# sinamalakouti/CDDMSL

Hardware: AMD Instinct MI355X
Metric: images/sec (train step) VOC+Clipart RN50-C4 (higher is better)
Workload: dtype bf16

## Files before the change

### cddmsl_amd/csrc/elementwise.hip

```cpp
#include "common.h"
#include <stdlib.h>

namespace {

template <typename T> struct Elt;
template <> struct Elt<__bf16> {
  static constexpr int ES = 2, VEC = 8;
  __device__ static __forceinline__ void unpack(const u32x4& v, float* f) {
#pragma unroll
    for (int j = 0; j < 4; ++j) { f[2 * j] = bf2f(v[j] & 0xffff); f[2 * j + 1] = bf2f(v[j] >> 16); }
  }
  __device__ static __forceinline__ u32x4 pack(const float* f) {
    u32x4 v;
#pragma unroll
    for (int j = 0; j < 4; ++j) v[j] = pack2bf(f[2 * j], f[2 * j + 1]);
    return v;
  }
  __device__ static __forceinline__ float ld(const char* p) { return bf2f(*(const unsigned short*)p); }
  __device__ static __forceinline__ void st(char* p, float v) { *(unsigned short*)p = f2bf(v); }
};
template <> struct Elt<float> {
  static constexpr int ES = 4, VEC = 4;
  __device__ static __forceinline__ void unpack(const u32x4& v, float* f) {
    const f32x4 x = __builtin_bit_cast(f32x4, v);
    f[0] = x[0]; f[1] = x[1]; f[2] = x[2]; f[3] = x[3];
  }
  __device__ static __forceinline__ u32x4 pack(const float* f) {
    f32x4 x = {f[0], f[1], f[2], f[3]};
    return __builtin_bit_cast(u32x4, x);
  }
  __device__ static __forceinline__ float ld(const char* p) { return *(const float*)p; }
  __device__ static __forceinline__ void st(char* p, float v) { *(float*)p = v; }
};

template <typename T>
__device__ __forceinline__ void preprocess_px(const unsigned char* img, char* out, int n, int h, int w, int Hp, int Wp, int Cp,
                                              float m0, float m1, float m2, float s0, float s1, float s2, float div) {
  long i = (long)blockIdx.x * blockDim.x + threadIdx.x;
  if (i >= (long)Hp * Wp) return;
  const unsigned ii = (unsigned)i;
  int x = ii % (unsigned)Wp, y = ii / (unsigned)Wp;
  float v[3] = {0.f, 0.f, 0.f};
  if (y < h && x < w) {
    long o = (long)y * w + x, pl = (long)h * w;
    v[0] = ((float)img[o] / div - m0) / s0;
    v[1] = ((float)img[pl + o] / div - m1) / s1;
    v[2] = ((float)img[2 * pl + o] / div - m2) / s2;
  }
  char* dst = out + (((long)n * Hp + y) * Wp + x) * Cp * Elt<T>::ES;
  if (Cp == Elt<T>::VEC) {
    float o[8] = {v[0], v[1], v[2], 0.f, 0.f, 0.f, 0.f, 0.f};
    *(u32x4*)dst = Elt<T>::pack(o);
    return;
// ... 320 lines not shown
  }
}

template <typename T>
__global__ void k_attnpool_softmax_fwd(const float* S, float* p, char* pT, long rows, int H, int P1, int TP, float scale) {
  const long r = (long)blockIdx.x * blockDim.x + threadIdx.x;
  if (r >= rows) return;
  const long k = r / H; const int h = (int)(r - k * H);
  const float* s = S + r * TP;
  float mx = -INFINITY;
  for (int t = 0; t < P1; ++t) mx = fmaxf(mx, s[t] * scale);
  float sum = 0.f;
  for (int t = 0; t < P1; ++t) sum += expf(s[t] * scale - mx);
  const float inv = 1.f / sum;
  for (int t = 0; t < TP; ++t) {
    float v = 0.f;
    if (t < P1) { v = expf(s[t] * scale - mx) * inv; p[r * P1 + t] = v; }
    Elt<T>::st(pT + ((k * TP + t) * H + h) * Elt<T>::ES, v);
  }
}
template <typename T>
__global__ void k_attnpool_softmax_bwd(const float* p, const float* dP, char* dsT, char* pds, long rows, int H, int P1, int TP,
                                       float scale) {
  const long r = (long)blockIdx.x * blockDim.x + threadIdx.x;
  if (r >= rows) return;
  const long k = r / H; const int h = (int)(r - k * H);
  const float* pr = p + r * P1;
  const float* dp = dP + r * TP;
  float dot = 0.f;
  for (int t = 0; t < P1; ++t) dot += pr[t] * dp[t];
  char* prow = pds + ((k * 2 * H + h) * TP) * Elt<T>::ES;
  char* drow = pds + ((k * 2 * H + H + h) * TP) * Elt<T>::ES;
  for (int t = 0; t < TP; ++t) {
    float pv = 0.f, ds = 0.f;
    if (t < P1) { pv = pr[t]; ds = pv * (dp[t] - dot) * scale; }
    Elt<T>::st(dsT + ((k * TP + t) * H + h) * Elt<T>::ES, ds);
    Elt<T>::st(prow + t * Elt<T>::ES, pv);
    Elt<T>::st(drow + t * Elt<T>::ES, ds);
  }
}

template <typename T>
__global__ __launch_bounds__(256) void k_attnpool_softmax_fwd_w(const float* __restrict__ S, float* __restrict__ p, char* __restrict__ pT,
                                                                long K, int H, int P1, int TP, float scale) {
  const long k = (long)blockIdx.x * 4 + (threadIdx.x >> 6);
  const int t = threadIdx.x & 63;
  if (k >= K) return;
  float v[32];
#pragma unroll
  for (int h = 0; h < 32; ++h) {
    v[h] = 0.f;
    if (h < H) {
      const bool in = t < P1;
      const float x = in ? S[(k * H + h) * TP + t] * scale : -INFINITY;
      const float mx = wave_max(x);
      const float e = in ? expf(x - mx) : 0.f;
      const float sum = wave_sum(e);
      v[h] = e * (1.f / sum);
      if (in) p[(k * H + h) * P1 + t] = v[h];
    }
  }
  if (t < TP) {
    char* dst = pT + ((k * TP + t) * H) * Elt<T>::ES;
    if (H % Elt<T>::VEC == 0) {
#pragma unroll
      for (int g = 0; g < 32 / Elt<T>::VEC; ++g)
        if (g * Elt<T>::VEC < H) ((u32x4*)dst)[g] = Elt<T>::pack(v + g * Elt<T>::VEC);
    } else {
#pragma unroll
      for (int h = 0; h < 32; ++h)
        if (h < H) Elt<T>::st(dst + h * Elt<T>::ES, v[h]);
    }
  }
}
template <typename T>
__global__ __launch_bounds__(256) void k_attnpool_softmax_bwd_w(const float* __restrict__ p, const float* __restrict__ dP,
                                                                char* __restrict__ dsT, char* __restrict__ pds, long K, int H, int P1,
                                                                int TP, float scale) {
  const long k = (long)blockIdx.x * 4 + (threadIdx.x >> 6);
  const int t = threadIdx.x & 63;
  if (k >= K) return;
  float dsv[32];
#pragma unroll
  for (int h = 0; h < 32; ++h) {
    dsv[h] = 0.f;
    if (h < H) {
      const bool in = t < P1;
      const float pv = in ? p[(k * H + h) * P1 + t] : 0.f;
      const float dp = in ? dP[(k * H + h) * TP + t] : 0.f;
      const float dot = wave_sum(pv * dp);
      dsv[h] = in ? pv * (dp - dot) * scale : 0.f;
      if (t < TP) {
        Elt<T>::st(pds + ((k * 2 * H + h) * TP + t) * Elt<T>::ES, pv);
        Elt<T>::st(pds + ((k * 2 * H + H + h) * TP + t) * Elt<T>::ES, dsv[h]);
      }
    }
  }
  if (t < TP) {
    char* dst = dsT + ((k * TP + t) * H) * Elt<T>::ES;
    if (H % Elt<T>::VEC == 0) {
#pragma unroll
      for (int g = 0; g < 32 / Elt<T>::VEC; ++g)
        if (g * Elt<T>::VEC < H) ((u32x4*)dst)[g] = Elt<T>::pack(dsv + g * Elt<T>::VEC);
    } else {
#pragma unroll
      for (int h = 0; h < 32; ++h)
        if (h < H) Elt<T>::st(dst + h * Elt<T>::ES, dsv[h]);
    }
  }
}

template <typename T>
__global__ void k_relu_bwd(const char* g, const char* y, char* dx, long nchunks, int g_f32) {
  for (long i = (long)blockIdx.x * blockDim.x + threadIdx.x; i < nchunks; i += (long)gridDim.x * blockDim.x) {
    float a[8], m[8], o[8];
    Elt<T>::unpack(((const u32x4*)y)[i], m);
    if (g_f32 && Elt<T>::VEC == 8) {
      Elt<float>::unpack(((const u32x4*)g)[2 * i], a);
      Elt<float>::unpack(((const u32x4*)g)[2 * i + 1], a + 4);
    } else Elt<T>::unpack(((const u32x4*)g)[i], a);
#pragma unroll
    for (int j = 0; j < Elt<T>::VEC; ++j) o[j] = m[j] > 0.f ? a[j] : 0.f;
    ((u32x4*)dx)[i] = Elt<T>::pack(o);
  }
}

template <typename T>
__global__ void k_colsum(const char* x, float* out, long rows, int cols, int period, int slab) {
  int c = blockIdx.x * 64 + (threadIdx.x & 63);
  int rlane = threadIdx.x >> 6;
  int res = blockIdx.z;
  long j0 = (long)blockIdx.y * slab;
  long nj = (rows - res + period - 1) / period;
  float s = 0.f;
  if (c < cols)
    for (long j = j0 + rlane; j < min(nj, j0 + slab); j += 4) s += Elt<T>::ld(x + ((res + period * j) * cols + c) * Elt<T>::ES);
  __shared__ float red[4][64];
  red[rlane][threadIdx.x & 63] = s;
  __syncthreads();
  if (rlane == 0 && c < cols) atomicAdd(out + (long)res * cols + c, red[0][threadIdx.x] + red[1][threadIdx.x] + red[2][threadIdx.x] + red[3][threadIdx.x]);
}

template <typename T>
__global__ void k_colsum_vec(const char* x, float* out, long rows, int cols, int period, int slab) {
// ... 469 lines not shown
```

### cddmsl_amd/hip.py

```python
import ctypes
import math
import os
from ctypes import c_float, c_int, c_long, c_void_p

import torch

from ._lib import check, lib, ptr, require_cuda, stream_ptr

DT = {torch.bfloat16: 0, torch.float32: 1}

_sigs_done = False


def _L():
    global _sigs_done
    L = lib()
    if not _sigs_done:
        vp, ci, cf = c_void_p, c_int, c_float
        L.cddmsl_last_kernel.argtypes = []
        L.cddmsl_plan_only.argtypes = [ci]
        L.cddmsl_conv_fwd.argtypes = [vp] * 7 + [ci] * 16 + [vp]
        L.cddmsl_bottleneck64_ok.argtypes = [ci] * 4
        L.cddmsl_bottleneck64_fwd.argtypes = [vp] * 17 + [ci] * 4 + [vp]
        L.cddmsl_conv_wgrad.argtypes = [vp] * 4 + [ci] * 12 + [vp]
        L.cddmsl_set_workspace.argtypes = [vp, c_long]
        L.cddmsl_weight_prep.argtypes = [vp] * 4 + [ci] * 5 + [vp]
        L.cddmsl_weight_prep_multi.argtypes = [vp, ci, ci, vp]
        L.cddmsl_preprocess.argtypes = [vp, vp] + [ci] * 6 + [vp, vp, ci, ci, vp]
        L.cddmsl_maxpool3s2_fwd.argtypes = [vp, vp] + [ci] * 5 + [vp]
        L.cddmsl_upsample_zero2.argtypes = [vp] * 4 + [ci] * 5 + [vp]
        L.cddmsl_meanpool_fwd.argtypes = [vp, vp, c_long, ci, ci, ci, vp]
        L.cddmsl_meanpool_bwd.argtypes = [vp, vp, c_long, ci, ci, ci, vp]
        L.cddmsl_preprocess224.argtypes = [vp, vp] + [ci] * 11 + [vp, vp, ci, vp]
        L.cddmsl_preprocess_batch.argtypes = [vp, vp, vp, ci, vp, ci, ci, ci, vp, vp, ci, ci, vp]
        L.cddmsl_preprocess224_batch.argtypes = [vp, vp, vp, ci, vp] + [ci] * 8 + [vp, vp, ci, vp]
        L.cddmsl_tta_view.argtypes = [vp] + [ci] * 4 + [vp, vp, vp, ci] * 2 + [vp, ci, ci, ci] * 2 + [ci, vp, vp, ci, ci, vp]
        L.cddmsl_resize_batch_u8.argtypes = [vp, c_long, vp, c_long, vp, c_long, vp, ci, vp]
        L.cddmsl_avgpool2_fwd.argtypes = [vp, vp] + [ci] * 5 + [vp]
        L.cddmsl_avgpool2_bwd.argtypes = [vp] * 4 + [ci] * 5 + [vp]
        L.cddmsl_avgpool2_bwd_q8.argtypes = [vp] * 4 + [ci] * 4 + [vp] * 4
        L.cddmsl_avgpool2_fwd_bits.argtypes = [vp] * 3 + [ci] * 5 + [vp]
        L.cddmsl_avgpool2_bwd_bits.argtypes = [vp] * 3 + [ci] * 5 + [vp]
        L.cddmsl_conv3x3_pool_fwd.argtypes = [vp] * 6 + [ci] * 7 + [vp]
        L.cddmsl_attn_tokens_fwd.argtypes = [vp] * 3 + [ci] * 5 + [vp]
        L.cddmsl_attn_tokens_bwd.argtypes = [vp] * 4 + [ci] * 5 + [vp]
        L.cddmsl_attnpool_softmax_fwd.argtypes = [vp] * 3 + [c_long, ci, ci, ci, cf, ci, vp]
        L.cddmsl_attnpool_softmax_bwd.argtypes = [vp] * 4 + [c_long, ci, ci, ci, cf, ci, vp]
        L.cddmsl_gemm_nt_batched.argtypes = [vp] * 4 + [ci] * 7 + [c_long] * 3 + [ci, ci, vp]
        L.cddmsl_gemm_tn_batched.argtypes = [vp] * 3 + [ci] * 7 + [c_long] * 3 + [ci, ci, vp]
        L.cddmsl_relu_bwd.argtypes = [vp, vp, vp, c_long, ci, ci, vp]
        L.cddmsl_colsum.argtypes = [vp, vp, c_long, ci, ci, ci, vp]
        L.cddmsl_sgd_clip_step.argtypes = [vp] * 4 + [ci, vp] + [cf] * 4 + [ci, vp]
        L.cddmsl_sgd_step_groups.argtypes = [vp] * 6 + [ci, vp, cf, ci, ci, cf, ci, vp]
        L.cddmsl_roi_align_forward.argtypes = [vp] * 5 + [ci] * 7 + [cf, ci, ci, ci, vp]
        L.cddmsl_roi_align_backward.argtypes = [vp] * 7 + [ci] * 7 + [cf, ci, ci, ci, vp]
        L.cddmsl_nms_anyorder.argtypes = [vp] * 4 + [ci, cf, vp, vp, vp]
        L.cddmsl_soft_nms.argtypes = [vp] * 6 + [ci, ci, cf, cf, cf, ci, vp, vp, vp]
        L.cddmsl_openset_logits.argtypes = [vp] * 4 + [ci] * 4 + [cf, cf, vp]
        L.cddmsl_openset_select.argtypes = [vp, vp, ci, vp, ci, vp, ci, ci, cf, cf, cf] + [vp] * 6 + [ci, vp, vp, vp]
        L.cddmsl_roi_align_nchw_anyorder.argtypes = [vp] * 3 + [ci] * 7 + [cf, ci, ci, ci, vp, vp, vp]
        L.cddmsl_roi_align_backward_nchw_anyorder.argtypes = [vp] * 3 + [ci] * 7 + [cf, ci, ci, ci, vp, vp, vp]
        L.cddmsl_quantize_fp8.argtypes = [vp] * 4 + [c_long, ci, vp]
        L.cddmsl_conv_fwd_fp8.argtypes = [vp] * 7 + [ci] * 10 + [vp] * 4
        L.cddmsl_conv_wgrad_fp8_ok.argtypes = [ci] * 6
        L.cddmsl_conv_wgrad_fp8.argtypes = [vp] * 4 + [ci] * 9 + [vp]
        L.cddmsl_conv_fwd_q8.argtypes = [vp] * 7 + [ci] * 10 + [vp] * 4
        L.cddmsl_fp8_dot_nt.argtypes = [vp] * 4 + [ci] * 4 + [vp]
        L.cddmsl_roi_align_forward_affine.argtypes = [vp] * 6 + [ci] * 8 + [cf, ci, ci, ci] + [vp] * 4
        L.cddmsl_roi_align_backward_pooled.argtypes = [vp] * 7 + [ci] * 7 + [cf, ci, ci, ci, vp]
        L.cddmsl_anchors.argtypes = [vp, vp, ci, ci, ci, cf, cf, vp]
        L.cddmsl_sort_desc.argtypes = [vp] * 5 + [ci, ci, vp, vp, vp]
        L.cddmsl_rpn_decode.argtypes = [vp] * 6 + [ci] * 5 + [cf] * 8 + [vp]
        L.cddmsl_nms.argtypes = [vp] * 5 + [ci, ci, cf, ci, vp]
        L.cddmsl_iou_match.argtypes = [vp, ci, vp, ci, vp, vp, vp, ci, cf, cf, ci, ci, ci, ci, vp]
        L.cddmsl_iou_match_batched.argtypes = [vp] * 7 + [ci] * 5 + [cf, cf] + [ci] * 4 + [vp]
        L.cddmsl_l2norm_fwd.argtypes = [vp, vp, vp, c_long, ci, cf, vp]
        L.cddmsl_l2norm_bwd.argtypes = [vp, vp, vp, vp, c_long, ci, vp]
        L.cddmsl_cosine_logits_fwd.argtypes = [vp] * 4 + [c_long, ci, ci, cf, cf, vp]
        L.cddmsl_cosine_logits_bwd.argtypes = [vp] * 5 + [c_long, ci, ci, cf, ci, vp]
        L.cddmsl_layernorm_fwd.argtypes = [vp] * 6 + [c_long, ci, cf, ci, vp]
        L.cddmsl_layernorm_bwd.argtypes = [vp] * 6 + [c_long, ci, ci, ci, vp]
        L.cddmsl_layernorm_bwd_emit.argtypes = [vp] * 7 + [c_long, ci, ci, ci, ctypes.POINTER(ci), vp]
        L.cddmsl_focal_ce_fwd.argtypes = [vp] * 4 + [c_long, ci, cf, ci, cf, vp]
        L.cddmsl_focal_ce_bwd.argtypes = [vp] * 5 + [c_long, ci, cf, ci, cf, vp]
        L.cddmsl_attn_small_fwd.argtypes = [vp] * 4 + [ci] * 8 + [cf, ci, vp]
        L.cddmsl_attn_small_bwd.argtypes = [vp] * 7 + [ci] * 8 + [cf, ci, vp]
        L.cddmsl_attn_tokens_fwd_mask.argtypes = [vp] * 4 + [ci] * 5 + [vp]
        L.cddmsl_attnpool_dx.argtypes = [vp] * 6 + [ci] * 6 + [vp]
        L.cddmsl_rpn_losses.argtypes = [vp, vp, vp, ci, vp, ci, vp, vp, vp, vp, c_long, cf, cf, cf, cf, cf, vp, vp, vp, vp, vp]
        L.cddmsl_box_l1.argtypes = [vp, ci, vp, ci, vp, vp, vp, cf, cf, cf, cf, cf, vp, vp, vp, vp]
        L.cddmsl_rpn_losses_reg.argtypes = [vp, vp, vp, ci, vp, ci, vp, vp, vp, vp, c_long, cf, cf, cf, cf, cf, ci, cf, cf, vp, vp, vp, vp, vp]
        L.cddmsl_box_reg_loss.argtypes = [vp, ci, vp, ci, vp, vp, vp, cf, cf, cf, cf, cf, ci, cf, cf, vp, vp, vp, vp]
        L.cddmsl_attn_last_fwd.argtypes = [vp] * 4 + [ci] * 8 + [cf, ci, vp]
        L.cddmsl_attn_last_bwd.argtypes = [vp] * 6 + [ci] * 8 + [cf, ci, vp]
        L.cddmsl_contrastive_fwd.argtypes = [vp] * 4 + [ci, ci, vp]
        L.cddmsl_contrastive_bwd.argtypes = [vp] * 5 + [ci, ci, vp]
        L.cddmsl_instance_boxes.argtypes = [vp] + [ci] * 4 + [vp, ci, vp, vp, vp, vp]
        L.cddmsl_text_embed.argtypes = [vp] * 4 + [c_long, ci, ci, ci, ci, vp]
        L.cddmsl_attn_causal_fwd.argtypes = [vp, vp] + [ci] * 6 + [cf, ci, vp]
        L.cddmsl_quick_gelu.argtypes = [vp, c_long, ci, vp]
# ... 648 lines not shown
def attnpool_dx_ok(K, H, P, TP, C, dtype):
    return dtype == torch.bfloat16 and P == 49 and TP == 56 and 2 * H <= 64 and (2 * H) % 8 == 0 and C % 128 == 0 and 0 < K <= 65535 * 8


@_timed("attnpool_dx")
def attnpool_dx(pds, zu, g0, mbits, P, gpos=None):
    require_cuda(pds, zu, g0, mbits)
    K, H2, TP = pds.shape
    C = zu.shape[2]
    assert pds.dtype == zu.dtype == torch.bfloat16 and g0.dtype == torch.float32 and mbits.dtype == torch.int64
    assert pds.is_contiguous() and zu.is_contiguous() and g0.is_contiguous() and mbits.is_contiguous() and tuple(zu.shape) == (K, H2, C)
    assert tuple(g0.shape) == (K, C) and tuple(mbits.shape) == (K, C) and (gpos is None or (gpos.dtype == torch.float32 and tuple(gpos.shape) == (P + 1, C) and gpos.is_contiguous()))
    dx = torch.empty((K, P, C), device=pds.device, dtype=pds.dtype)
    check(_L().cddmsl_attnpool_dx(ptr(pds), ptr(zu), ptr(g0), ptr(mbits), ptr(dx), ptr(gpos), K, H2, P, TP, C, 0, stream_ptr()), "cddmsl_attnpool_dx")
    return dx


@_timed("attn_tokens_bwd")
def attn_tokens_bwd(dtok, P, relu_mask=None, gpos=None, want_dx=True):
    require_cuda(dtok, relu_mask, gpos)
    K, TP, C = dtok.shape
    assert dtok.is_contiguous()
    assert relu_mask is None or (relu_mask.is_contiguous() and relu_mask.dtype == dtok.dtype and relu_mask.numel() == K * P * C)
    assert gpos is None or (gpos.is_contiguous() and gpos.dtype == torch.float32 and tuple(gpos.shape) == (P + 1, C))
    assert want_dx or gpos is not None
    dx = torch.empty((K, P, C), device=dtok.device, dtype=dtok.dtype) if want_dx else None
    check(_L().cddmsl_attn_tokens_bwd(ptr(dtok), ptr(relu_mask), ptr(dx), ptr(gpos), K, P, TP, C, _dt(dtok), stream_ptr()), "cddmsl_attn_tokens_bwd")
    return dx


@_timed("attnpool_softmax")
def attnpool_softmax_fwd(S, P1, scale, dtype):
    require_cuda(S)
    K, H, TP = S.shape
    assert S.dtype == torch.float32 and S.is_contiguous() and P1 <= TP
    p = torch.empty((K, H, P1), device=S.device, dtype=torch.float32)
    pT = torch.empty((K, TP, H), device=S.device, dtype=dtype)
    check(_L().cddmsl_attnpool_softmax_fwd(ptr(S), ptr(p), ptr(pT), K, H, P1, TP, float(scale), DT[dtype], stream_ptr()), "cddmsl_attnpool_softmax_fwd")
    return p, pT


@_timed("attnpool_softmax")
def attnpool_softmax_bwd(p, dP, scale, dtype):
    require_cuda(p, dP)
    K, H, P1 = p.shape
    TP = dP.shape[2]
    assert p.dtype == dP.dtype == torch.float32 and p.is_contiguous() and dP.is_contiguous() and dP.shape[:2] == (K, H)
    dsT = torch.empty((K, TP, H), device=p.device, dtype=dtype)
    pds = torch.empty((K, 2 * H, TP), device=p.device, dtype=dtype)
    check(_L().cddmsl_attnpool_softmax_bwd(ptr(p), ptr(dP), ptr(dsT), ptr(pds), K, H, P1, TP, float(scale), DT[dtype], stream_ptr()), "cddmsl_attnpool_softmax_bwd")
    return dsT, pds


def _eptr(t, elem_offset=0):
    return ctypes.c_void_p(t.data_ptr() + elem_offset * t.element_size())


@_timed("gemm_nt_batched")
def gemm_nt_batched(a, w, c, M, N, K, lda, ldb, ldc, batch, sa, sw, sc, a_off=0, w_off=0, c_off=0, bias=None):
    require_cuda(a, w, c, bias)
    assert a.dtype == w.dtype and c.dtype in (a.dtype, torch.float32)
    out_f32 = int(c.dtype == torch.float32 and a.dtype != torch.float32)
    check(_L().cddmsl_gemm_nt_batched(_eptr(a, a_off), _eptr(w, w_off), _eptr(c, c_off), ptr(bias), M, N, K, lda, ldb, ldc, batch,
                                      sa, sw, sc, out_f32, _dt(a), stream_ptr()), "cddmsl_gemm_nt_batched")


@_timed("gemm_tn_batched")
def gemm_tn_batched(a, b, out, M, N, K, lda, ldb, ldo, batch, sa, sb, so, a_off=0, b_off=0, o_off=0, accumulate=False):
    require_cuda(a, b, out)
    assert a.dtype == b.dtype
    if accumulate:
        assert out.dtype == torch.float32
        mode = 0
    else:
        mode = 1 if (out.dtype == torch.float32 and a.dtype != torch.float32) else (1 if out.dtype == torch.float32 else 2)
        assert out.dtype in (a.dtype, torch.float32)
    check(_L().cddmsl_gemm_tn_batched(_eptr(a, a_off), _eptr(b, b_off), _eptr(out, o_off), M, N, K, lda, ldb, ldo, batch, sa, sb, so,
                                      mode, _dt(a), stream_ptr()), "cddmsl_gemm_tn_batched")


@_timed("relu_bwd")
def relu_bwd(g, y):
    require_cuda(g, y)
    assert g.is_contiguous() and y.is_contiguous() and g.numel() == y.numel()
    g_f32 = int(g.dtype == torch.float32 and y.dtype != torch.float32)
    assert g_f32 or g.dtype == y.dtype
    dx = torch.empty_like(y)
    check(_L().cddmsl_relu_bwd(ptr(g), ptr(y), ptr(dx), y.numel(), g_f32, _dt(y), stream_ptr()), "cddmsl_relu_bwd")
    return dx


@_timed("colsum")
def colsum(x2d, period=1, out=None):
    require_cuda(x2d, out)
    rows, cols = x2d.shape
    assert x2d.is_contiguous()
    if out is None:
        out = torch.zeros((period, cols) if period > 1 else (cols,), device=x2d.device, dtype=torch.float32)
    check(_L().cddmsl_colsum(ptr(x2d), ptr(out), rows, cols, period, _dt(x2d), stream_ptr()), "cddmsl_colsum")
    return out


def same_layout(a, b):
    return a.shape == b.shape and all(sa == sb for sa, sb, n in zip(a.stride(), b.stride(), a.shape) if n > 1)


# ... 815 lines not shown
```

### cddmsl_amd/layers.py

```python
import os
import weakref

import torch

from . import hip

_STEP = [0]


def bump_weight_version():
    _STEP[0] += 1


_LOAD_GEN = [0]


def note_weights_loaded(*_):
    _LOAD_GEN[0] += 1
    _STEP[0] += 1


def load_generation():
    return _LOAD_GEN[0]

# ... 810 lines not shown
        shape, scale, sr, aligned, K = ctx.meta
        dy = dy.contiguous()
        dx = hip.roi_align_backward(dy[:K], rois, roi_start, shape, scale, sr, aligned)
        dextra = dy[K:] if (dy.shape[0] > K and ctx.needs_input_grad[8]) else None
        return dx, None, None, None, None, None, None, None, dextra


def roi_align(x, rois, roi_start, out_size, scale, sampling_ratio, aligned=True, with_pooled=False, extra=None):
    assert rois.dim() == 2 and rois.size(1) == 5
    assert extra is None or tuple(extra.shape[1:]) == (out_size, out_size, x.shape[3])
    if with_pooled and out_size % 2 == 0:
        y, yp = RoIAlignFn.apply(x, rois, roi_start, out_size, scale, sampling_ratio, aligned, True, extra)
        y._pooled2 = yp
        return y
    return RoIAlignFn.apply(x, rois, roi_start, out_size, scale, sampling_ratio, aligned, False, extra)


class AttnPoolParams:
    def __init__(self, pos, q_w, q_b, k_w, k_b, v_w, v_b, c_w, c_b, heads, frozen=False):
        self.pos, self.heads, self.frozen = pos, heads, frozen
        self.q_w, self.q_b, self.k_w, self.k_b, self.v_w, self.v_b, self.c_w, self.c_b = q_w, q_b, k_w, k_b, v_w, v_b, c_w, c_b
        self.pq = PreparedWeight(q_w, None, frozen)
        self.pk = PreparedWeight(k_w, None, frozen)
        self.pv = PreparedWeight(v_w, None, frozen)
        self.pc = PreparedWeight(c_w, None, frozen)


class AttnPoolFn(torch.autograd.Function):

    TP = 56

    @staticmethod
    def forward(ctx, x, anchor, ap, premask_input_grad=False):
        ctx.relu_src = x if premask_input_grad else None
        T = x.dtype
        K, h, w, C = x.shape
        P, TP, H = h * w, AttnPoolFn.TP, ap.heads
        D = C // H
        assert ap.pos.shape[0] == P + 1 <= TP, "attention pool needs a 7x7 map (clip_backbone.py:86)"
        dev = x.device
        fused_dx = hip.attnpool_dx_ok(K, H, P, TP, C, T) and bool(ctx.needs_input_grad[0]) and os.environ.get("CDDMSL_ATTNPOOL_DX", "1") != "0"
        mbits = None
        if fused_dx and premask_input_grad:
            tok, mbits = hip.attn_tokens_fwd_mask(x.view(K, P, C), ap.pos.detach(), TP)
        else:
            tok = hip.attn_tokens_fwd(x.view(K, P, C), ap.pos.detach(), TP)
        wq, _ = ap.pq.get(T, False)
        wk, wkT = ap.pk.get(T, True)
        wv, wvT = ap.pv.get(T, True)
        wc, _ = ap.pc.get(T, False)
        q0 = hip.conv_fwd(tok.view(K, 1, TP, C), wq, None, ap.q_b.detach(), stride=TP).view(K, C)
        zu = torch.empty((K, 2 * H, C), device=dev, dtype=T)
        hip.gemm_nt_batched(q0, wkT, zu, K, C, D, C, C, 2 * H * C, H, D, D, C, c_off=H * C)
        S = torch.empty((K, H, TP), device=dev, dtype=torch.float32)
        hip.gemm_nt_batched(zu, tok, S, H, TP, C, C, C, TP, K, 2 * H * C, TP * C, H * TP, a_off=H * C)
        p, pT = hip.attnpool_softmax_fwd(S, P + 1, D ** -0.5, T)
        z = torch.empty((K, H, C), device=dev, dtype=T)
        hip.gemm_tn_batched(pT, tok, z, TP, H, C, H, C, C, K, TP * H, TP * C, H * C)
        o = torch.empty((K, C), device=dev, dtype=T)
        hip.gemm_nt_batched(z, wv, o, K, D, C, H * C, C, C, H, C, D * C, D)
        o = o + ap.v_b.detach().to(T)
        out = hip.conv_fwd(o.view(1, 1, K, C), wc, None, ap.c_b.detach(), out_f32=True).view(K, -1)
        ctx.ap = ap
        ctx.fused_dx = fused_dx
        ctx.save_for_backward(tok, q0, zu, p, z, o, mbits)
        ctx.shape = (K, h, w, C)
        return out

    @staticmethod
    def backward(ctx, dout):
        ap = ctx.ap
        tok, q0, zu, p, z, o, mbits = ctx.saved_tensors
        K, h, w, C = ctx.shape
        P, TP, H = h * w, AttnPoolFn.TP, ap.heads
        D = C // H
        T = tok.dtype
        dev = tok.device
        train = not ap.frozen
        dout_t = dout.contiguous().to(T)
        if train:
            hip.conv_wgrad(o.view(1, 1, K, C), dout_t.view(1, 1, K, -1), _ohwi(ap.c_w).shape, out=_ohwi(_grad_buf(ap.c_w)))
            hip.colsum(dout_t, out=_grad_buf(ap.c_b))
        _, wcd = ap.pc.get(T, True)
        wk, wkT = ap.pk.get(T, True)
        wv, wvT = ap.pv.get(T, True)
        do = hip.conv_fwd(dout_t.view(1, 1, K, -1), wcd).view(K, C)
        if train:
            hip.colsum(do, out=_grad_buf(ap.v_b))
            hip.gemm_tn_batched(do, z, _grad_buf(ap.v_w), K, D, C, C, H * C, C, H, D, C, D * C, accumulate=True)
        hip.gemm_nt_batched(do, wvT, zu, K, C, D, C, C, 2 * H * C, H, D, D, C)
        dP = torch.empty((K, H, TP), device=dev, dtype=torch.float32)
        hip.gemm_nt_batched(zu, tok, dP, H, TP, C, C, C, TP, K, 2 * H * C, TP * C, H * TP)
        dsT, pds = hip.attnpool_softmax_bwd(p, dP, D ** -0.5, T)
        du = torch.empty((K, H, C), device=dev, dtype=T)
        hip.gemm_tn_batched(dsT, tok, du, TP, H, C, H, C, C, K, TP * H, TP * C, H * C)
        dq0 = torch.empty((K, C), device=dev, dtype=T)
        hip.gemm_nt_batched(du, wk, dq0, K, D, C, H * C, C, C, H, C, D * C, D)
        if train:
            hip.gemm_tn_batched(q0, du, _grad_buf(ap.k_w), K, D, C, C, H * C, C, H, D, C, D * C, accumulate=True)
            _grad_buf(ap.k_b)
            hip.conv_wgrad(tok.view(K, 1, TP, C), dq0.view(K, 1, 1, C), _ohwi(ap.q_w).shape, stride=TP, out=_ohwi(_grad_buf(ap.q_w)))
            hip.colsum(dq0, out=_grad_buf(ap.q_b))
        _, wqd = ap.pq.get(T, True)
        gpos = _grad_buf(ap.pos) if train else None
        want_dx = ctx.needs_input_grad[0]
        if ctx.fused_dx and want_dx:
            g0 = hip.conv_fwd(dq0.view(1, 1, K, C), wqd, out_f32=True).view(K, C)
            if mbits is None:
                mbits = torch.full((K, C), -1, device=dev, dtype=torch.int64)
            dx = hip.attnpool_dx(pds, zu, g0, mbits, P, gpos)
            return dx.view(K, h, w, C), None, None, None
        dtok = torch.empty((K, TP, C), device=dev, dtype=T)
        hip.gemm_tn_batched(pds, zu, dtok, 2 * H, TP, C, TP, C, C, K, 2 * H * TP, 2 * H * C, TP * C)
        dtok[:, 0, :] += hip.conv_fwd(dq0.view(1, 1, K, C), wqd).view(K, C)
        dx = None
        if want_dx or train:
            dx = hip.attn_tokens_bwd(dtok, P, ctx.relu_src if want_dx else None, gpos, want_dx)
        return (dx.view(K, h, w, C) if want_dx else None), None, None, None


def attnpool(x, ap):
    return AttnPoolFn.apply(x, None if ap.frozen else ap.q_w, ap)


_FP8_CONST = {}


def _fp8_const(value, device):
    k = (float(value), str(device))
    if k not in _FP8_CONST:
        _FP8_CONST[k] = torch.tensor([float(value)], device=device, dtype=torch.float32)
    return _FP8_CONST[k]


def fp8_unit_rows(wn):
    return hip.quantize_fp8(wn.contiguous(), _fp8_const(hip.FP8_MAX, wn.device))


class CosineLogitsFn(torch.autograd.Function):
    @staticmethod
    def forward(ctx, x, wn, temperature, fp8=False, wn8=None):
        x = x.contiguous()
        if fp8 and x.shape[1] % 64 == 0 and wn.shape[0] <= 32:
            xn, inv = hip.l2norm_fwd(x, 1e-12)
            unit = _fp8_const(hip.FP8_MAX, x.device)
            if wn8 is None:
                wn8 = fp8_unit_rows(wn)
            dot = hip.fp8_dot_nt(hip.quantize_fp8(xn, unit), wn8, _fp8_const(1.0 / (hip.FP8_MAX * hip.FP8_MAX * temperature), x.device))
# ... 305 lines not shown
```

### include/cddmsl_hip.h

```cpp
#ifndef CDDMSL_HIP_H
#define CDDMSL_HIP_H
#include <stddef.h>

#ifdef __cplusplus
extern "C" {
#endif

int cddmsl_abi_version(void);

int cddmsl_conv_fwd(const void* x, const void* w, void* y, const float* scale, const float* bias, const void* residual,
                    const void* relu_mask, int Nimg, int Hi, int Wi, int Cin, int Cout, int KH, int KW, int stride, int pad,
                    int pool, int ldy, int ldr, int ldm, int relu, int out_f32, int dtype, void* stream);
int cddmsl_conv3x3_pool_fwd(const void* x, const void* w, void* y, const float* scale, const float* bias, const void* relu_mask,
                            int Nimg, int Hi, int Wi, int Cin, int Cout, int stride, int dtype, void* stream);
int cddmsl_bottleneck64_ok(int Nimg, int H, int W, int dtype);
int cddmsl_bottleneck64_fwd(const void* o1, const void* w2, const float* s2, const float* b2, const void* w3, const float* s3,
                            const float* b3, const void* residual, const void* x0, const void* wd, const float* sd,
                            const float* bd, const void* w1n, const float* s1n, const float* b1n, void* out, void* o1n,
                            int Nimg, int H, int W, int dtype, void* stream);
int cddmsl_set_workspace(void* ptr, long bytes);
int cddmsl_conv_wgrad(const void* x, const void* dy, float* dw, const float* scale, int Nimg, int Hi, int Wi, int Cin,
                      int Cout, int KH, int KW, int stride, int pad, int pool, int ldd, int dtype, void* stream);
int cddmsl_gemm_nt_batched(const void* a, const void* w, void* c, const float* bias, int M, int N, int K, int lda, int ldb, int ldc,
                           int batch, long sa, long sw, long sc, int out_f32, int dtype, void* stream);
// ... 23 lines not shown
                              int* ws_fp, int N, int C, int H, int W, int K, int ph, int pw, float spatial_scale,
                              int sampling_ratio, int aligned, int dtype, void* stream);
int cddmsl_roi_align_forward_affine(const void* x, const float* rois, void* y, void* y_pooled, const float* scale,
                                    const float* bias, int relu, int N, int C, int H, int W, int K, int ph, int pw,
                                    float spatial_scale, int sampling_ratio, int aligned, int dtype, void* y8, const float* q8,
                                    float* amax8, void* stream);
int cddmsl_roi_align_backward_pooled(const void* dy, const float* rois, const int* roi_start, void* dx, float* ws_ay,
                                     float* ws_ax, int* ws_fp, int N, int C, int H, int W, int K, int ph, int pw,
                                     float spatial_scale, int sampling_ratio, int aligned, int dtype, void* stream);
int cddmsl_roi_align_nchw_anyorder(const void* input, const float* rois, void* output, int N, int C, int H, int W, int K, int ph, int pw,
                                   float spatial_scale, int sampling_ratio, int aligned, int dtype, void* temp, size_t* temp_bytes,
                                   void* stream);
int cddmsl_roi_align_backward_nchw_anyorder(const void* grad, const float* rois, void* grad_input, int N, int C, int H, int W, int K,
                                            int ph, int pw, float spatial_scale, int sampling_ratio, int aligned, int dtype, void* temp,
                                            size_t* temp_bytes, void* stream);

int cddmsl_anchors(const float* cell, float* out, int Hf, int Wf, int A, float stride, float offset, void* stream);
int cddmsl_sort_desc(const float* keys_in, float* keys_out, int* idx_scratch, int* order_out, const int* offsets, int N,
                     int total, void* temp, size_t* temp_bytes, void* stream);
int cddmsl_rpn_decode(const int* order, const float* deltas, const float* cell, const int* img_hw, float* boxes,
                      unsigned char* valid, int N, int Hf, int Wf, int A, int topk, float stride, float offset, float wx,
                      float wy, float ww, float wh, float scale_clamp, float min_size, void* stream);
int cddmsl_nms(const float* boxes, const unsigned char* valid, unsigned long long* mask_ws, int* keep, int* nkeep, int N,
               int n, float thr, int max_keep, void* stream);
int cddmsl_nms_anyorder(const float* boxes, const float* scores, long* keep, int* nkeep, int K, float iou_threshold, void* temp,
                        size_t* temp_bytes, void* stream);
int cddmsl_soft_nms(const float* boxes, const float* scores, const long* idxs, long* keep, float* keep_scores, int* nkeep, int K,
                    int method, float sigma, float iou_threshold, float prune_threshold, int max_keep, void* temp,
                    size_t* temp_bytes, void* stream);
int cddmsl_openset_logits(const float* x, const float* wn, float* logits, float* stats, int R, int D, int K, int ld,
                          float temperature, float eps, void* stream);
int cddmsl_openset_select(const float* logits, const float* stats, int ld, const float* boxes, int ldb, const float* objectness,
                          int R, int K, float img_h, float img_w, float score_thresh, int* cand_row, int* cand_cls,
                          float* cand_score, float* cand_box, unsigned char* valid, int* count, int cap, void* temp,
                          size_t* temp_bytes, void* stream);
int cddmsl_iou_match(const float* gt, int G, const float* preds, int P, long* matches, signed char* labels,
                     unsigned int* best_ws, int nthr, float t0, float t1, int l0, int l1, int l2, int allow_low_quality,
                     void* stream);

int cddmsl_iou_match_batched(const float* gt, const int* gt_off, const float* preds, const int* pred_off, long* matches,
                             signed char* labels, unsigned int* best_ws, int N, int P, int maxG, int totalG, int nthr, float t0,
                             float t1, int l0, int l1, int l2, int allow_low_quality, void* stream);

int cddmsl_attn_tokens_fwd(const void* x, const float* pos, void* tok, int K, int P, int TP, int C, int dtype, void* stream);
int cddmsl_attn_tokens_fwd_mask(const void* x, const float* pos, void* tok, unsigned long long* mbits, int K, int P, int TP, int C,
                                int dtype, void* stream);
int cddmsl_attnpool_dx(const void* pds, const void* zu, const float* g0, const unsigned long long* mbits, void* dx, float* gpos, int K,
                       int H2, int P, int TP, int C, int dtype, void* stream);
int cddmsl_attn_tokens_bwd(const void* dtok, const void* relu_mask, void* dx, float* gpos, int K, int P, int TP, int C, int dtype,
                           void* stream);
int cddmsl_attnpool_softmax_fwd(const float* S, float* p, void* pT, long K, int H, int P1, int TP, float scale, int dtype, void* stream);
int cddmsl_attnpool_softmax_bwd(const float* p, const float* dP, void* dsT, void* pds, long K, int H, int P1, int TP, float scale,
                                int dtype, void* stream);

int cddmsl_attn_small_fwd(const void* q, const void* k, const void* v, void* o, int nseq, int t, int heads, int dh, int ldq,
                          int ldk, int ldv, int ldo, float scale, int dtype, void* stream);
int cddmsl_attn_small_bwd(const void* q, const void* k, const void* v, const void* dout, void* dq, void* dk, void* dv, int nseq,
                          int t, int heads, int dh, int ldq, int ldk, int ldv, int ldo, float scale, int dtype, void* stream);
int cddmsl_attn_last_fwd(const void* q, const void* kv, void* o, float* p, int n, int t, int heads, int dh, int ldq, int ldkv, int voff,
                         int ldo, float scale, int dtype, void* stream);
int cddmsl_attn_last_bwd(const void* q, const void* kv, const void* dout, const float* p, void* dq, void* dkv, int n, int t, int heads,
                         int dh, int ldq, int ldkv, int voff, int ldo, float scale, int dtype, void* stream);

int cddmsl_text_embed(const long* ids, const void* tok, const float* pos, float* x, long rows, int t, int W, int vocab, int dtype,
                      void* stream);
int cddmsl_attn_causal_fwd(const void* qkv, void* o, int nseq, int t, int heads, int dh, int ldqkv, int ldo, float scale, int dtype,
                           void* stream);
int cddmsl_quick_gelu(void* x, long numel, int dtype, void* stream);
int cddmsl_text_pool(const float* x, const long* rows, const float* gamma, const float* beta, void* y, long R, int nout, int group,
                     int W, float eps, int dtype, void* stream);

int cddmsl_skinny_gemm_workspace(int M, int N, int K);
int cddmsl_skinny_gemm(const void* x, const void* w, const float* bias, const float* residual, void* y, float* ws, long ws_bytes, int M,
                       int N, int K, int epi, void* stream);
int cddmsl_lm_head_workspace(int M, int V);
int cddmsl_lm_head_argmax(const void* h, const void* wte, long* ids, int ld_ids, float* logits, void* ws, long ws_bytes, int M, int V,
                          int K, void* stream);
int cddmsl_decode_attn(const void* qkv, void* kc, void* vc, void* o, int nseq, int heads, int dh, int L, int Lmax, int ldqkv, float scale,
                       int dtype, void* stream);
int cddmsl_pos_embed(const long* ids, int ld_ids, const void* tab, const float* src, const float* wpe, float* x, long rows, int t, int pos0,
                     int W, int vocab, int npos, int dtype, void* stream);
int cddmsl_gelu_new(void* x, long numel, int dtype, void* stream);
int cddmsl_lm_head_topk_workspace(int M, int V);
int cddmsl_lm_head_topk(const void* h, const void* wte, float* vals, int* idx, float* logZ, float* logits, void* ws, long ws_bytes, int M,
                        int V, int K, int B, void* stream);
int cddmsl_beam_step(const float* vals, const int* idx, const float* logZ, const float* sum_in, const int* len_in,
                     const unsigned char* stop_in, const int* hist_in, const unsigned char* anc_in, float* sum_out, int* len_out,
                     unsigned char* stop_out, int* hist_out, unsigned char* anc_out, int* src, long* next_tok, int n, int B, int T, int step,
                     int stop_id, void* stream);
int cddmsl_decode_attn_beam(const void* qkv, const void* pk, const void* pv, void* gk, void* gv, const unsigned char* anc, void* o, int rows,
                            int B, int heads, int dh, int P, int L, int Tg, int ldanc, int ldqkv, float scale, int dtype, void* stream);

int cddmsl_l2norm_fwd(const float* x, float* y, float* inv, long R, int D, float eps, void* stream);
int cddmsl_l2norm_bwd(const float* dy, const float* y, const float* inv, float* dx, long R, int D, void* stream);
int cddmsl_cosine_logits_fwd(const float* x, const float* wn, float* scores, float* inv, long R, int D, int Kc,
                             float temperature, float eps, void* stream);
int cddmsl_cosine_logits_bwd(const float* ds, const float* x, const float* wn, const float* inv, float* dx, long R, int D,
                             int Kc, float temperature, int accumulate, void* stream);
int cddmsl_layernorm_fwd(const float* x, const float* gamma, const float* beta, void* y, float* mean, float* rstd, long R, int D,
                         float eps, int dtype, void* stream);
int cddmsl_layernorm_bwd(const void* dy, const float* x, const float* gamma, const float* mean, const float* rstd, float* dx,
                         long R, int D, int accumulate, int dtype, void* stream);
int cddmsl_layernorm_bwd_emit(const void* dy, const float* x, const float* gamma, const float* mean, const float* rstd, float* dx,
                              void* dx_bf16, long R, int D, int accumulate, int dtype, int* emitted, void* stream);
int cddmsl_focal_ce_fwd(const float* logits, const long* target, float* row_loss, float* probs, long R, int C, float gamma,
                        int bg_class, float bg_weight, void* stream);
// ... 62 lines not shown
```

Before: 167.9.

## Fuse attention-pool score GEMM, softmax and value GEMM into one persistent kernel

Adds a persistent HIP kernel that, for each pooled region, computes the head-by-token scores with MFMA, applies the softmax (or its backward) in registers and LDS, then multiplies by the token matrix through an LDS ring buffer filled by async global-to-LDS loads. It replaces three launches (score GEMM, softmax kernel, value GEMM) in both forward and backward, and removes the fp32 score tensor and transposed probability tensor round-trips through memory. The path is limited to bf16 with H=32, P1=50, TP=56 and C a multiple of 256, and can be turned off with an environment variable. The softmax math is moved into a shared header and reused by the old kernels.

```diff
diff --git a/cddmsl_amd/csrc/attnpool_fused.hip b/cddmsl_amd/csrc/attnpool_fused.hip
--- /dev/null
+++ b/cddmsl_amd/csrc/attnpool_fused.hip
@@ -0,0 +1,241 @@
+#include "gemm_common.h"
+#include "attnpool_softmax.h"
+
+namespace {
+
+constexpr int AF_H = 32, AF_P1 = 50, AF_TP = 56;
+constexpr int AF_STAGE = 16384;
+constexpr int AF_PB = AF_H * 64 * 2;
+constexpr int AF_NST = 4, AF_RING = AF_NST * AF_STAGE;
+constexpr int AF_WG_PER_CU = 2;
+
+struct AttnFusedArgs {
+  const char* a;
+  const char* tok;
+  float* p;
+  char* pds;
+  char* out;
+  long sa;
+  int K, C, bpb;
+  float scale;
+};
+
+template <int N>
+__device__ __forceinline__ void af_wait_vm() { asm volatile("s_waitcnt vmcnt(%0)" :: "n"(N) : "memory"); }
+
+template <int NST>
+__device__ __forceinline__ void af_wait_younger(int groups, int stages) {
+  static_assert((NST - 1) * 20 <= 63 && NST <= 4, "vmcnt is a 6-bit field");
+  switch (groups * 4 + stages) {
+#define CDDMSL_AF_W(G, S) case (G) * 4 + (S): af_wait_vm<(G) * 16 + (S) * 4>(); break;
+#define CDDMSL_AF_WG(G) CDDMSL_AF_W(G, 0) CDDMSL_AF_W(G, 1) CDDMSL_AF_W(G, 2) CDDMSL_AF_W(G, 3)
+    CDDMSL_AF_WG(0) CDDMSL_AF_WG(1) CDDMSL_AF_WG(2)
+    CDDMSL_AF_W(3, 0) CDDMSL_AF_W(3, 1) CDDMSL_AF_W(3, 2) CDDMSL_AF_W(3, 3)
+#undef CDDMSL_AF_WG
+#undef CDDMSL_AF_W
+    default: af_wait_vm<0>(); break;
+  }
+}
+
+template <bool BWD, int UN>
+__global__ __launch_bounds__(256, AF_WG_PER_CU) void k_attnpool_fused(AttnFusedArgs p) {
+  constexpr int H = AF_H, P1 = AF_P1, TP = AF_TP;
+  constexpr int NST = AF_NST, RING = AF_RING;
+  __shared__ __attribute__((aligned(16))) char lds[RING + AF_PB];
+  float* const part = (float*)lds;
+  unsigned short* const pb = (unsigned short*)(lds + RING);
+  const int t = threadIdx.x, lane = t & 63, r = lane & 31, h = lane >> 5;
+  const int wv = __builtin_amdgcn_readfirstlane(t >> 6);
+  const int cw = p.C >> 2, ns = cw >> 4;
+  const int nsl = p.C >> 7;
+  const long b0 = (long)blockIdx.x * p.bpb;
+  const int nreg = (int)min((long)p.bpb, (long)p.K - b0);
+  const char* zp = (const char*)g_zero_page;
+  const unsigned lbase = (unsigned)(size_t)(__attribute__((address_space(3))) char*)lds;
+  unsigned xoff0, xoff1;
+  {
+    const int g = lane >> 4, li = lane & 15, q = li >> 2, pp = li & 3, hh = g >> 1;
+    const int ch = ((wv * 32 + 16 * (g & 1)) >> 3) + (pp >> 1);
+    const int r0 = 8 * hh + q, r1 = r0 + 4;
+    xoff0 = r0 * 256 + 16 * (ch ^ fsw(r0)) + 8 * (pp & 1);
+    xoff1 = r1 * 256 + 16 * (ch ^ fsw(r1)) + 8 * (pp & 1);
+  }
+
+#pragma unroll 1
+  for (int reg = 0; reg < nreg; ++reg) {
+    const long k = b0 + reg;
+    int C = p.C;
+    asm volatile("" : "+s"(C));
+    const char* tokk = p.tok + k * ((long)TP * C * 2);
+    f32x16 s0, s1;
+#pragma unroll
+    for (int g = 0; g < 16; ++g) { s0[g] = 0.f; s1[g] = 0.f; }
+    {
+      const char* ub = p.a + k * p.sa;
+      const unsigned lo = (unsigned)(r * C + wv * cw + h * 8) * 2u;
+      const unsigned lo1 = (unsigned)(min(r + 32, P1 - 1) * C + wv * cw + h * 8) * 2u;
+      u32x4 au[UN], a0[UN], a1[UN], bu[UN], b0[UN], b1[UN];
+      auto ld = [&](u32x4* u, u32x4* x0, u32x4* x1, int s) {
+#pragma unroll
+        for (int j = 0; j < UN; ++j) {
+          const unsigned so = (unsigned)min(s + j, ns - 1) * 32u;
+          u[j] = *(const u32x4*)(ub + (lo + so));
+          x0[j] = *(const u32x4*)(tokk + (lo + so));
+          x1[j] = *(const u32x4*)(tokk + (lo1 + so));
+        }
+      };
+      auto mm = [&](const u32x4* u, const u32x4* x0, const u32x4* x1) {
+#pragma unroll
+        for (int j = 0; j < UN; ++j) {
+          Mma<__bf16>::step(s0, u[j], x0[j]);
+          Mma<__bf16>::step(s1, u[j], x1[j]);
+        }
+      };
+      ld(au, a0, a1, 0);
+#pragma unroll 1
+      for (int s = 0; s < ns; s += 2 * UN) {
+        ld(bu, b0, b1, s + UN);
+        __builtin_amdgcn_sched_barrier(0);
+        mm(au, a0, a1);
+        __builtin_amdgcn_sched_barrier(0);
+        ld(au, a0, a1, s + 2 * UN);
+        __builtin_amdgcn_sched_barrier(0);
+        mm(bu, b0, b1);
+        __builtin_amdgcn_sched_barrier(0);
+      }
+    }
+#pragma unroll
+    for (int g = 0; g < 16; ++g) {
+      const int hd = (g & 3) + 8 * (g >> 2) + 4 * h;
+      part[(wv * H + hd) * 64 + r] = s0[g];
+      part[(wv * H + hd) * 64 + 32 + r] = s1[g];
+    }
+    __syncthreads();
+    {
+      const bool in = lane < P1;
+      float sv[8], v[8], pv[8];
+#pragma unroll
+      for (int i = 0; i < 8; ++i) {
+        const int hd = wv * 8 + i;
+        const float x = ((part[hd * 64 + lane] + part[(H + hd) * 64 + lane]) + part[(2 * H + hd) * 64 + lane]) + part[(3 * H + hd) * 64 + lane];
+        sv[i] = in ? x : 0.f;
+      }
+      float* prow = p.p + (k * H + wv * 8) * P1;
+      if (!BWD) {
+        attnpool_softmax_rows<8>(sv, in, p.scale, v);
+#pragma unroll
+        for (int i = 0; i < 8; ++i)
+          if (in) prow[i * P1 + lane] = v[i];
+      } else {
+#pragma unroll
+        for (int i = 0; i < 8; ++i) pv[i] = in ? prow[i * P1 + lane] : 0.f;
+        attnpool_softmax_rows_bwd<8>(pv, sv, in, p.scale, v);
+        unsigned short* drow = (unsigned short*)p.pds + (k * 2 * H + wv * 8) * TP;
+        if (lane < TP) {
+#pragma unroll
+          for (int i = 0; i < 8; ++i) {
+            drow[i * TP + lane] = f2bf(pv[i]);
+            drow[(H + i) * TP + lane] = f2bf(v[i]);
+          }
+        }
+      }
+#pragma unroll
+      for (int i = 0; i < 8; ++i) pb[(wv * 8 + i) * 64 + lane] = f2bf(v[i]);
+    }
+    __syncthreads();
+    u32x4 fa[4];
+#pragma unroll
+    for (int ms = 0; ms < 4; ++ms) fa[ms] = *(const u32x4*)(lds + RING + r * 128 + ms * 32 + h * 16);
+    f32x16 acc;
+#pragma unroll
+    for (int g = 0; g < 16; ++g) acc[g] = 0.f;
+    char* outk = p.out + k * ((long)H * C * 2);
+    const unsigned vo = (unsigned)(wv * 32 + r) * 2u + (unsigned)h * 8u * (unsigned)C;
+    int tt = t;
+    asm volatile("" : "+v"(tt));
+    const int xr = tt >> 4, xc = (tt & 15) ^ fsw(tt >> 4);
+    const unsigned xo = (unsigned)xc * 16u + (unsigned)xr * 2u * (unsigned)C;
+    auto stage = [&](int slot, int sl) {
+      char* base = lds + slot * AF_STAGE;
+      const char* xb = tokk + (long)sl * 256;
+#pragma unroll
+      for (int i = 0; i < 4; ++i) {
+        const char* src = xb + (xo + (unsigned)i * 32u * (unsigned)C);
+        glds16((i < 3 || xr + 48 < P1) ? src : zp, base + (i * 256 + wv * 64) * 16);
+      }
+    };
+#pragma unroll
+    for (int i = 0; i < NST - 1; ++i)
+      if (i < nsl) stage(i, i);
+#pragma unroll 1
+    for (int it = 0; it < nsl; ++it) {
+      const int slot = it % NST;
+      if (it + NST - 1 < nsl) stage((it + NST - 1) % NST, it + NST - 1);
+      af_wait_younger<NST>(min(it, NST - 1), min(NST - 1, nsl - 1 - it));
+      __builtin_amdgcn_s_barrier();
+      const unsigned x0 = lbase + slot * AF_STAGE + xoff0, x1 = lbase + slot * AF_STAGE + xoff1;
+#define CDDMSL_AF_TRS(DST, IMM)                                                                  \
+  { u32x2 q0_, q1_;                                                                              \
+    asm volatile("ds_read_b64_tr_b16 %0, %1 offset:%2" : "=v"(q0_) : "v"(x0), "i"(IMM));         \
+    asm volatile("ds_read_b64_tr_b16 %0, %1 offset:%2" : "=v"(q1_) : "v"(x1), "i"(IMM));         \
+    DST = u32x4{q0_[0], q0_[1], q1_[0], q1_[1]}; }
+      u32x4 fb[4];
+      CDDMSL_AF_TRS(fb[0], 0) CDDMSL_AF_TRS(fb[1], 4096) CDDMSL_AF_TRS(fb[2], 8192) CDDMSL_AF_TRS(fb[3], 12288)
+#undef CDDMSL_AF_TRS
+      asm volatile("s_waitcnt lgkmcnt(0)" : "+v"(fb[0]), "+v"(fb[1]), "+v"(fb[2]), "+v"(fb[3]) :: "memory");
+      __builtin_amdgcn_sched_barrier(0);
+#pragma unroll
+      for (int ms = 0; ms < 4; ++ms) Mma<__bf16>::step(acc, fa[ms], fb[ms]);
+      __builtin_amdgcn_s_barrier();
+      char* o = outk + (long)it * 256;
+#pragma unroll
+      for (int g = 0; g < 16; ++g) {
+        Mma<__bf16>::store(o + (long)((g & 3) + 8 * (g >> 2)) * C * 2 + vo, acc[g]);
+        acc[g] = 0.f;
+      }
+    }
+  }
+}
+
+bool attnpool_sv_contract(int K, int H, int P1, int TP, int C, int dtype) {
+  return dtype == 0 && K >= 0 && H == AF_H && P1 == AF_P1 && TP == AF_TP && C > 0 && C % 256 == 0 && C <= 65536;
+}
+
+int attnpool_sv_run(int K) {
+  int cus = persistent_blocks_raw();
+  if (cus <= 0) cus = 256;
+  const int slots = cus * AF_WG_PER_CU;
+  return (K + slots - 1) / slots;
+}
+
+template <bool BWD>
+void attnpool_sv_launch(AttnFusedArgs& a, hipStream_t st) {
+  a.bpb = attnpool_sv_run(a.K);
+  const dim3 grid((unsigned)((a.K + a.bpb - 1) / a.bpb));
+  if (a.C % 512 == 0) hipLaunchKernelGGL((k_attnpool_fused<BWD, 4>), grid, dim3(256), 0, st, a);
+  else hipLaunchKernelGGL((k_attnpool_fused<BWD, 2>), grid, dim3(256), 0, st, a);
+}
+
+}
+
+extern "C" int cddmsl_attnpool_sv_fwd(const void* zu, const void* tok, float* p, void* z, int K, int H, int P1, int TP, int C, float scale,
+                                      int dtype, void* stream) {
+  if (!attnpool_sv_contract(K, H, P1, TP, C, dtype) || !zu || !tok || !p || !z) return CDDMSL_ERR_ARG;
+  if (K == 0) return CDDMSL_OK;
+  AttnFusedArgs a;
+  a.a = (const char*)zu + (long)H * C * 2; a.tok = (const char*)tok; a.p = p; a.pds = nullptr; a.out = (char*)z;
+  a.sa = (long)2 * H * C * 2; a.K = K; a.C = C; a.scale = scale;
+  attnpool_sv_launch<false>(a, (hipStream_t)stream);
+  return launch_status();
+}
+
+extern "C" int cddmsl_attnpool_sv_bwd(const void* zu, const void* tok, const float* p, void* pds, void* du, int K, int H, int P1, int TP,
+                                      int C, float scale, int dtype, void* stream) {
+  if (!attnpool_sv_contract(K, H, P1, TP, C, dtype) || !zu || !tok || !p || !pds || !du) return CDDMSL_ERR_ARG;
+  if (K == 0) return CDDMSL_OK;
+  AttnFusedArgs a;
+  a.a = (const char*)zu; a.tok = (const char*)tok; a.p = (float*)p; a.pds = (char*)pds; a.out = (char*)du;
+  a.sa = (long)2 * H * C * 2; a.K = K; a.C = C; a.scale = scale;
+  attnpool_sv_launch<true>(a, (hipStream_t)stream);
+  return launch_status();
+}
diff --git a/cddmsl_amd/csrc/attnpool_softmax.h b/cddmsl_amd/csrc/attnpool_softmax.h
--- /dev/null
+++ b/cddmsl_amd/csrc/attnpool_softmax.h
@@ -0,0 +1,47 @@
+#pragma once
+#include "common.h"
+
+template <int N>
+__device__ __forceinline__ void attnpool_softmax_rows(const float (&s)[N], bool in, float scale, float (&p)[N]) {
+  float x[N], mx[N], e[N], sum[N];
+#pragma unroll
+  for (int i = 0; i < N; ++i) { x[i] = in ? s[i] * scale : -INFINITY; mx[i] = x[i]; }
+#pragma unroll
+  for (int o = 32; o > 0; o >>= 1)
+#pragma unroll
+    for (int i = 0; i < N; ++i) mx[i] = fmaxf(mx[i], __shfl_xor(mx[i], o, 64));
+#pragma unroll
+  for (int i = 0; i < N; ++i) { e[i] = in ? expf(x[i] - mx[i]) : 0.f; sum[i] = e[i]; }
+#pragma unroll
+  for (int o = 32; o > 0; o >>= 1)
+#pragma unroll
+    for (int i = 0; i < N; ++i) sum[i] += __shfl_xor(sum[i], o, 64);
+#pragma unroll
+  for (int i = 0; i < N; ++i) p[i] = e[i] * (1.f / sum[i]);
+}
+
+template <int N>
+__device__ __forceinline__ void attnpool_softmax_rows_bwd(const float (&pv)[N], const float (&dp)[N], bool in, float scale, float (&ds)[N]) {
+  float dot[N];
+#pragma unroll
+  for (int i = 0; i < N; ++i) dot[i] = pv[i] * dp[i];
+#pragma unroll
+  for (int o = 32; o > 0; o >>= 1)
+#pragma unroll
+    for (int i = 0; i < N; ++i) dot[i] += __shfl_xor(dot[i], o, 64);
+#pragma unroll
+  for (int i = 0; i < N; ++i) ds[i] = in ? pv[i] * (dp[i] - dot[i]) * scale : 0.f;
+}
+
+__device__ __forceinline__ float attnpool_softmax_row(float s, bool in, float scale) {
+  const float a[1] = {s};
+  float p[1];
+  attnpool_softmax_rows<1>(a, in, scale, p);
+  return p[0];
+}
+__device__ __forceinline__ float attnpool_softmax_row_bwd(float pv, float dp, bool in, float scale) {
+  const float a[1] = {pv}, b[1] = {dp};
+  float ds[1];
+  attnpool_softmax_rows_bwd<1>(a, b, in, scale, ds);
+  return ds[0];
+}
diff --git a/cddmsl_amd/csrc/elementwise.hip b/cddmsl_amd/csrc/elementwise.hip
--- a/cddmsl_amd/csrc/elementwise.hip
+++ b/cddmsl_amd/csrc/elementwise.hip
@@ -1,4 +1,5 @@
 #include "common.h"
+#include "attnpool_softmax.h"
 #include <stdlib.h>
 
 namespace {
@@ -425,11 +426,7 @@
     v[h] = 0.f;
     if (h < H) {
       const bool in = t < P1;
-      const float x = in ? S[(k * H + h) * TP + t] * scale : -INFINITY;
-      const float mx = wave_max(x);
-      const float e = in ? expf(x - mx) : 0.f;
-      const float sum = wave_sum(e);
-      v[h] = e * (1.f / sum);
+      v[h] = attnpool_softmax_row(in ? S[(k * H + h) * TP + t] : 0.f, in, scale);
       if (in) p[(k * H + h) * P1 + t] = v[h];
     }
   }
@@ -461,8 +458,7 @@
       const bool in = t < P1;
       const float pv = in ? p[(k * H + h) * P1 + t] : 0.f;
       const float dp = in ? dP[(k * H + h) * TP + t] : 0.f;
-      const float dot = wave_sum(pv * dp);
-      dsv[h] = in ? pv * (dp - dot) * scale : 0.f;
+      dsv[h] = attnpool_softmax_row_bwd(pv, dp, in, scale);
       if (t < TP) {
         Elt<T>::st(pds + ((k * 2 * H + h) * TP + t) * Elt<T>::ES, pv);
         Elt<T>::st(pds + ((k * 2 * H + H + h) * TP + t) * Elt<T>::ES, dsv[h]);
diff --git a/cddmsl_amd/hip.py b/cddmsl_amd/hip.py
--- a/cddmsl_amd/hip.py
+++ b/cddmsl_amd/hip.py
@@ -46,6 +46,8 @@
         L.cddmsl_attn_tokens_bwd.argtypes = [vp] * 4 + [ci] * 5 + [vp]
         L.cddmsl_attnpool_softmax_fwd.argtypes = [vp] * 3 + [c_long, ci, ci, ci, cf, ci, vp]
         L.cddmsl_attnpool_softmax_bwd.argtypes = [vp] * 4 + [c_long, ci, ci, ci, cf, ci, vp]
+        L.cddmsl_attnpool_sv_fwd.argtypes = [vp] * 4 + [ci] * 5 + [cf, ci, vp]
+        L.cddmsl_attnpool_sv_bwd.argtypes = [vp] * 5 + [ci] * 5 + [cf, ci, vp]
         L.cddmsl_gemm_nt_batched.argtypes = [vp] * 4 + [ci] * 7 + [c_long] * 3 + [ci, ci, vp]
         L.cddmsl_gemm_tn_batched.argtypes = [vp] * 3 + [ci] * 7 + [c_long] * 3 + [ci, ci, vp]
         L.cddmsl_relu_bwd.argtypes = [vp, vp, vp, c_long, ci, ci, vp]
@@ -800,6 +802,42 @@
     return dsT, pds
 
 
+def attnpool_fused_ok(K, H, P1, TP, C, dtype):
+    return (dtype == torch.bfloat16 and H == 32 and P1 == 50 and TP == 56 and C % 256 == 0 and 0 < C <= 65536 and K >= 0
+            and os.environ.get("CDDMSL_ATTNPOOL_FUSED", "1") != "0")
+
+
+def _attnpool_fused_bytes(K, H, P1, TP, C, bwd):
+    return float(K * (2 * H * C * 2 + P1 * C * 2 + H * P1 * 4 + (2 * H * TP * 2 if bwd else 0)))
+
+
+def attnpool_sv_fwd(zu, tok, P1, scale):
+    require_cuda(zu, tok)
+    K, H2, C = zu.shape
+    H, TP = H2 // 2, tok.shape[1]
+    assert zu.dtype == tok.dtype == torch.bfloat16 and zu.is_contiguous() and tok.is_contiguous() and tuple(tok.shape) == (K, TP, C)
+    p = torch.empty((K, H, P1), device=zu.device, dtype=torch.float32)
+    z = torch.empty((K, H, C), device=zu.device, dtype=zu.dtype)
+    e0 = PROFILE.begin("attnpool_fused")
+    check(_L().cddmsl_attnpool_sv_fwd(ptr(zu), ptr(tok), ptr(p), ptr(z), K, H, P1, TP, C, float(scale), 0, stream_ptr()), "cddmsl_attnpool_sv_fwd")
+    PROFILE.end(e0, "attnpool_fused", 2.0 * K * H * C * (TP + P1), nbytes=_attnpool_fused_bytes(K, H, P1, TP, C, False))
+    return p, z
+
+
+def attnpool_sv_bwd(zu, tok, p, scale):
+    require_cuda(zu, tok, p)
+    K, H2, C = zu.shape
+    H, TP, P1 = H2 // 2, tok.shape[1], p.shape[2]
+    assert zu.dtype == tok.dtype == torch.bfloat16 and p.dtype == torch.float32 and zu.is_contiguous() and tok.is_contiguous() and p.is_contiguous()
+    assert tuple(tok.shape) == (K, TP, C) and tuple(p.shape) == (K, H, P1)
+    pds = torch.empty((K, H2, TP), device=zu.device, dtype=zu.dtype)
+    du = torch.empty((K, H, C), device=zu.device, dtype=zu.dtype)
+    e0 = PROFILE.begin("attnpool_fused")
+    check(_L().cddmsl_attnpool_sv_bwd(ptr(zu), ptr(tok), ptr(p), ptr(pds), ptr(du), K, H, P1, TP, C, float(scale), 0, stream_ptr()), "cddmsl_attnpool_sv_bwd")
+    PROFILE.end(e0, "attnpool_fused", 2.0 * K * H * C * (TP + P1), nbytes=_attnpool_fused_bytes(K, H, P1, TP, C, True))
+    return pds, du
+
+
 def _eptr(t, elem_offset=0):
     return ctypes.c_void_p(t.data_ptr() + elem_offset * t.element_size())
 
diff --git a/cddmsl_amd/layers.py b/cddmsl_amd/layers.py
--- a/cddmsl_amd/layers.py
+++ b/cddmsl_amd/layers.py
@@ -886,11 +886,14 @@
         q0 = hip.conv_fwd(tok.view(K, 1, TP, C), wq, None, ap.q_b.detach(), stride=TP).view(K, C)
         zu = torch.empty((K, 2 * H, C), device=dev, dtype=T)
         hip.gemm_nt_batched(q0, wkT, zu, K, C, D, C, C, 2 * H * C, H, D, D, C, c_off=H * C)
-        S = torch.empty((K, H, TP), device=dev, dtype=torch.float32)
-        hip.gemm_nt_batched(zu, tok, S, H, TP, C, C, C, TP, K, 2 * H * C, TP * C, H * TP, a_off=H * C)
-        p, pT = hip.attnpool_softmax_fwd(S, P + 1, D ** -0.5, T)
-        z = torch.empty((K, H, C), device=dev, dtype=T)
-        hip.gemm_tn_batched(pT, tok, z, TP, H, C, H, C, C, K, TP * H, TP * C, H * C)
+        if hip.attnpool_fused_ok(K, H, P + 1, TP, C, T):
+            p, z = hip.attnpool_sv_fwd(zu, tok, P + 1, D ** -0.5)
+        else:
+            S = torch.empty((K, H, TP), device=dev, dtype=torch.float32)
+            hip.gemm_nt_batched(zu, tok, S, H, TP, C, C, C, TP, K, 2 * H * C, TP * C, H * TP, a_off=H * C)
+            p, pT = hip.attnpool_softmax_fwd(S, P + 1, D ** -0.5, T)
+            z = torch.empty((K, H, C), device=dev, dtype=T)
+            hip.gemm_tn_batched(pT, tok, z, TP, H, C, H, C, C, K, TP * H, TP * C, H * C)
         o = torch.empty((K, C), device=dev, dtype=T)
         hip.gemm_nt_batched(z, wv, o, K, D, C, H * C, C, C, H, C, D * C, D)
         o = o + ap.v_b.detach().to(T)
@@ -923,11 +926,14 @@
             hip.colsum(do, out=_grad_buf(ap.v_b))
             hip.gemm_tn_batched(do, z, _grad_buf(ap.v_w), K, D, C, C, H * C, C, H, D, C, D * C, accumulate=True)
         hip.gemm_nt_batched(do, wvT, zu, K, C, D, C, C, 2 * H * C, H, D, D, C)
-        dP = torch.empty((K, H, TP), device=dev, dtype=torch.float32)
-        hip.gemm_nt_batched(zu, tok, dP, H, TP, C, C, C, TP, K, 2 * H * C, TP * C, H * TP)
-        dsT, pds = hip.attnpool_softmax_bwd(p, dP, D ** -0.5, T)
-        du = torch.empty((K, H, C), device=dev, dtype=T)
-        hip.gemm_tn_batched(dsT, tok, du, TP, H, C, H, C, C, K, TP * H, TP * C, H * C)
+        if hip.attnpool_fused_ok(K, H, P + 1, TP, C, T):
+            pds, du = hip.attnpool_sv_bwd(zu, tok, p, D ** -0.5)
+        else:
+            dP = torch.empty((K, H, TP), device=dev, dtype=torch.float32)
+            hip.gemm_nt_batched(zu, tok, dP, H, TP, C, C, C, TP, K, 2 * H * C, TP * C, H * TP)
+            dsT, pds = hip.attnpool_softmax_bwd(p, dP, D ** -0.5, T)
+            du = torch.empty((K, H, C), device=dev, dtype=T)
+            hip.gemm_tn_batched(dsT, tok, du, TP, H, C, H, C, C, K, TP * H, TP * C, H * C)
         dq0 = torch.empty((K, C), device=dev, dtype=T)
         hip.gemm_nt_batched(du, wk, dq0, K, D, C, H * C, C, C, H, C, D * C, D)
         if train:
diff --git a/include/cddmsl_hip.h b/include/cddmsl_hip.h
--- a/include/cddmsl_hip.h
+++ b/include/cddmsl_hip.h
@@ -99,6 +99,10 @@
 int cddmsl_attnpool_softmax_fwd(const float* S, float* p, void* pT, long K, int H, int P1, int TP, float scale, int dtype, void* stream);
 int cddmsl_attnpool_softmax_bwd(const float* p, const float* dP, void* dsT, void* pds, long K, int H, int P1, int TP, float scale,
                                 int dtype, void* stream);
+int cddmsl_attnpool_sv_fwd(const void* zu, const void* tok, float* p, void* z, int K, int H, int P1, int TP, int C, float scale,
+                           int dtype, void* stream);
+int cddmsl_attnpool_sv_bwd(const void* zu, const void* tok, const float* p, void* pds, void* du, int K, int H, int P1, int TP, int C,
+                           float scale, int dtype, void* stream);
 
 int cddmsl_attn_small_fwd(const void* q, const void* k, const void* v, void* o, int nseq, int t, int heads, int dh, int ldq,
                           int ldk, int ldv, int ldo, float scale, int dtype, void* stream);
```

Result: no change. 168.5, median of 3 (+0.4%).
